# decisiongraph/duckdb-annsearch

Hardware: AMD Instinct MI355X
Metric: queries/sec @ recall@10>=0.95, 10Mx768 fp32, batch=1024 (higher is better)
Workload: dtype f32 results (fp16-image certified filter + exact fp32 rerank); 1 GPU; FAISS IVFFlat nlist=1024 nprobe=32, 10000000x768 fp32 (low-rank gaussian, intrinsic dim 16, noise 0.02), batch=1024, k=10; global_batch=1024, n=10000000, d=768, k=10, parallelism=shard1

## Files before the change

### duckdb-annsearch_amd/csrc/ivf.cpp

```cpp
#include "../../include/hip_ann.h"
#include "ivf.hpp"

#include <algorithm>
#include <chrono>
#include <cstdio>
#include <cstdlib>
#include <cstring>
#include <exception>
#include <numeric>

using namespace hipann;

namespace {

void set_err(char *buf, int len, const char *msg) {
    if (!buf || len <= 0) return;
    std::strncpy(buf, msg, (size_t)len - 1);
    buf[len - 1] = '\0';
}

template <typename F>
int guard_int(char *eb, int el, F &&f) {
    try {
        return f();
// ... 471 lines not shown
    int *cand_i = nullptr;
    const float *qn = nullptr;
    if (form != kFormDirect && metric == kL2) {
        const FlatShard &qs = *sh.quant->shards[0];
        if (probes_in && img) {
            qn = qsh0.qn.get<float>();
        } else if (!probes_in && qs.qn_of == xq && qs.qn_nq == nq) {
            qn = qs.qn.get<float>();
        } else {
            sh.qn.ensure(sizeof(float) * (size_t)nq, sh.device);
            launch_row_norms(xq, nq, d, sh.qn.get<float>(), st);
            qn = sh.qn.get<float>();
        }
    }
    if (tiled && !img) ensure_tiled_codes(sh, d, nlist, st);
    if (img) {
    } else if (ivf_form_split(form)) {
        sh.qsplit.ensure((size_t)ivf_mfma_bf_qsplit_bytes(nq, d, ivf_form_terms(form)), sh.device);
    }
    {
        RoctxRange rr("hipann.ivf.scan");
        ScopedTiming t(ix.timer_main, st);
        if (img) {
            auto scan_h = [&](int phase, const int *slots, int64_t items, float *pd, int *pi, int subl) {
                launch_ivf_scan_mfma_h(nq, i8 ? sh.qi8.p : sh.hsplit.p, i8 ? sh.qs8.get<float>() : sh.hits.get<float>(),
                                       i8 ? sh.qres8.get<float>() : sh.hres.get<float>(), cert8 ? sh.qhn2.get<float>() : qn, d,
                                       metric, i8 ? sh.codes_i8.p : sh.codes_h.p, sh.tpass_off.get<int64_t>(), sh.xnorm.get<float>(),
                                       sh.list_off.get<int64_t>(), sh.list_len.get<int>(), sh.cnt.get<int>(), sh.bucket_off.get<int>(),
                                       sh.item_off.get<int>(), sh.bucket.get<int>(), slots, nlist, np, k,
                                       items, qbound, pd, pi, st, subl,
                                       i8 ? 1 : 0, i8 ? sh.xs8.get<float>() : nullptr,
                                       cert8 ? sh.xr8.get<float>() : nullptr, cert8 ? sh.qhn.get<float>() : nullptr, phase,
                                       sh.goff.get<int>());
            };
            if (seeded) {
                HIPANN_REQUIRE((int64_t)np * nq * sh.max_nch + nq < (int64_t)0x7fffffff, "too many candidate slots");
                sh.cslot.ensure(sizeof(int) * (size_t)nq * np, sh.device);
                sh.bcnt.ensure(sizeof(int) * (size_t)nq, sh.device);
                cand_d = sh.part_d.get<float>() + (size_t)np * nq * kslot;
                cand_i = sh.part_i.get<int>() + (size_t)np * nq * kslot;
                scan_h(1, nullptr, ivf_max_items(nq, np, nlist, 1, 0, group), sh.part_d.get<float>(), sh.part_i.get<int>(), 1);
                launch_ivf_seed_bound(sh.part_d.get<float>(), sh.part_i.get<int>(), sh.slot_off.get<int>(), np, nq, kslot,
                                      sh.n, qbound, cand_d, cand_i, sh.cslot.get<int>(), sh.bcnt.get<int>(), st);
                scan_h(2, sh.cslot.get<int>(), ivf_max_items(nq, np, nlist, sh.max_nch - 1, sh.n, group), cand_d, cand_i, 1);
            } else {
                scan_h(0, sh.slot_off.get<int>(), max_items, sh.part_d.get<float>(), sh.part_i.get<int>(), sub ? 1 : 0);
            }
        }
        else if (bigk)
            launch_ivf_scan_bigk(xq, d, metric, sh.codes, sh.list_off.get<int64_t>(), sh.list_len.get<int>(),
                                 sh.coarse_i.get<int64_t>(),
                                 nq * np, np, sh.slot_off.get<int>(), nq * np * std::max(sh.max_nch, 1), k,
                                 sh.part_d.get<float>(), sh.part_i.get<int>(), st);
        else if (ivf_form_split(form))
            launch_ivf_scan_mfma_bf(ivf_form_terms(form), xq, nq, sh.qsplit.p, qn, d, metric, sh.codes_t.get<float>(),
                                    sh.tpass_off.get<int64_t>(), sh.xnorm.get<float>(), sh.list_off.get<int64_t>(),
                                    sh.list_len.get<int>(), sh.cnt.get<int>(), sh.bucket_off.get<int>(), sh.item_off.get<int>(),
                                    sh.bucket.get<int>(), sh.slot_off.get<int>(), nlist, np, k, max_items, qbound,
                                    sh.part_d.get<float>(), sh.part_i.get<int>(), st, sub ? 1 : 0);
        else if (form == kFormDecomposed)
            launch_ivf_scan_mfma(xq, qn, d, metric, sh.codes_t.get<float>(), sh.tpass_off.get<int64_t>(),
                                 sh.xnorm.get<float>(), sh.list_off.get<int64_t>(), sh.list_len.get<int>(),
                                 sh.cnt.get<int>(),
                                 sh.bucket_off.get<int>(), sh.item_off.get<int>(), sh.bucket.get<int>(),
                                 sh.slot_off.get<int>(), nlist, np, k, max_items, qbound, sh.part_d.get<float>(),
                                 sh.part_i.get<int>(), st);
        else
// ... 20 lines not shown
        fb_maxch = sh.max_nch;
        const size_t per_f = (size_t)np * fb_maxch * kout * (sizeof(float) + sizeof(long long));
        fb_cap = (int)std::min<int64_t>({nq, 64, std::max<int64_t>(1, (int64_t)(((size_t)64 << 20) / per_f))});
        sh.fbc_d.ensure(sizeof(float) * (size_t)fb_cap * np * fb_maxch * kout, sh.device);
        sh.fbc_i.ensure(sizeof(long long) * (size_t)fb_cap * np * fb_maxch * kout, sh.device);
        if (sh.fbc_cap < fb_cap || !sh.fbc_done.p) {
            sh.fbc_done.ensure(sizeof(unsigned) * (size_t)std::max(fb_cap, 64), sh.device);
            HIPANN_CHECK(hipMemsetAsync(sh.fbc_done.p, 0, sh.fbc_done.bytes, st));
            sh.fbc_cap = (int)(sh.fbc_done.bytes / sizeof(unsigned));
        }
    }
    {
        RoctxRange rr("hipann.ivf.rerank");
        ScopedTiming t(ix.timer_merge, st);
        launch_ivf_rerank(seeded ? cand_d : sh.part_d.get<float>(), seeded ? cand_i : sh.part_i.get<int>(),
                          sh.slot_off.get<int>(), np, nq, kfilt, kout,
                          metric, xq, sh.codes, d, sh.ids, sh.n, 0, xmax2, D, I, sh.nflag.get<int>(),
                          sh.flagged.get<int>(), st, kSplit2Eps, i8 ? rxmax8 : half ? sh.half_rxmax : -1.f,
                          i8 ? sh.qres8.get<float>() : half ? sh.hres.get<float>() : nullptr, sh.coarse_i.get<int64_t>(),
                          sh.list_off.get<int64_t>(), nlist, qbound, img && metric == kL2 ? qn : nullptr, kslot,
                          sub ? 1 : 0, inline_fb ? sh.list_len.get<int>() : nullptr,
                          inline_fb ? sh.fpd.get<float>() : nullptr, inline_fb ? sh.fpi.get<long long>() : nullptr,
                          inline_fb ? sh.fb_total.get<unsigned long long>() : nullptr, fb_cap, cert8 ? 1 : 0,
                          seeded ? sh.bcnt.get<int>() : nullptr);
        if (fb_cap > 0)
            launch_ivf_fallback_chunks(sh.nflag.get<int>(), sh.flagged.get<int>(), fb_cap, np, fb_maxch, ivf_chunk_rows(),
                                       kout, metric, xq, sh.codes, d, sh.ids, 0, sh.coarse_i.get<int64_t>(),
                                       sh.list_off.get<int64_t>(), sh.list_len.get<int>(), nlist, sh.fbc_d.get<float>(),
                                       sh.fbc_i.get<long long>(), sh.fbc_done.get<unsigned>(), D, I,
                                       sh.fb_total.get<unsigned long long>(), st,
                                       as_half && !probation ? auto8_host_word(sh) : nullptr, (unsigned)++sh.fb_seq);
    }
    if (sh.count_only) return;
    if (probation) auto8_probation(ix, sh, nq, xq, k_user, kout, st, probes_in);
    if (inline_fb) return;
    int nf = 0;
    HIPANN_CHECK(hipMemcpyAsync(&nf, sh.nflag.p, sizeof(int), hipMemcpyDeviceToHost, st));
    HIPANN_CHECK(hipStreamSynchronize(st));
    if (nf <= 0) return;
    ix.rerank_fallbacks += nf;
    const size_t pbytes = sizeof(int64_t) * (size_t)nq * np;
    sh.coarse_save.ensure(pbytes, sh.device);
    HIPANN_CHECK(hipMemcpyAsync(sh.coarse_save.p, sh.coarse_i.p, pbytes, hipMemcpyDeviceToDevice, st));
    sh.fq.ensure(sizeof(float) * (size_t)nf * d, sh.device);
    sh.fD.ensure(sizeof(float) * (size_t)nf * kout, sh.device);
    sh.fI.ensure(sizeof(int64_t) * (size_t)nf * kout, sh.device);
    launch_ivf_gather_queries(xq, sh.flagged.get<int>(), nf, d, sh.fq.get<float>(), st);
// ... 834 lines not shown
```

### duckdb-annsearch_amd/csrc/ivf_kernels.hip

```cpp
#include "common.hpp"
#include "wave_topk.hpp"

#include <algorithm>
#include <cstdlib>
#include <utility>

namespace hipann {

constexpr int IVF_WAVES = 8;
constexpr int IVF_THREADS = 64 * IVF_WAVES;
constexpr int IVF_G = 32;
constexpr int IVF_QW = IVF_G / IVF_WAVES;
constexpr int IVF_TR = 256;
constexpr int IVF_BK = 24;
constexpr int IVF_LD = IVF_BK + 4;
#ifndef HIPANN_IVF_CH
#define HIPANN_IVF_CH 2048
#endif
constexpr int IVF_CH = HIPANN_IVF_CH;

__device__ __forceinline__ int ivf_nch(int len) { return (len + IVF_CH - 1) / IVF_CH; }

__global__ void ivf_count(const int64_t *__restrict__ probes, int64_t npairs, const int *__restrict__ list_len,
                          int nlist, int *__restrict__ cnt) {
// ... 1775 lines not shown
#endif
template <bool IP, int WV>
__global__ void __launch_bounds__(WV == 1 ? 256 : 64 * WV, WV == 4 ? HIPANN_RR_MINB : 1)
ivf_rerank_topk(const float *__restrict__ pd, const int *__restrict__ pi, const int *__restrict__ slot_off,
                int nprobe, int64_t nq, int k, int kout, const float *__restrict__ Q,
                const float *__restrict__ codes, int d, const int64_t *__restrict__ ids, int64_t nrows,
                int64_t label_offset, float xmax2, float *__restrict__ D, int64_t *__restrict__ I,
                int *__restrict__ nflag, int *__restrict__ flagged, float eps, float rxmax,
                const float *__restrict__ qres, const int64_t *__restrict__ probes,
                const int64_t *__restrict__ list_off, int nlist, const unsigned *__restrict__ qbound,
                const float *__restrict__ qnorm, int kslot, int sub, const int *__restrict__ list_len,
                float *__restrict__ fpd, long long *__restrict__ fpi, unsigned long long *__restrict__ fb_total,
                int fb_cap, int i8_l2, const int *__restrict__ seed_cnt) {
    const int64_t q = WV == 1 ? (int64_t)blockIdx.x * 4 + (threadIdx.x >> 6) : (int64_t)blockIdx.x;
    if (q >= nq) return;
    const int lane = threadIdx.x & 63;
    const int wv = WV == 1 ? 0 : (int)(threadIdx.x >> 6);
    RR_STAMP(0);
    long long rr_t = HIPANN_RR_PROF ? clock64() : 0;
    WaveList<1, int> L;
    L.init();
    const int64_t s0 = slot_off ? slot_off[q * nprobe] : q * nprobe;
    const int64_t s1 = slot_off ? slot_off[(q + 1) * nprobe] : (q + 1) * nprobe;
    const int64_t total = seed_cnt ? kSeedK + (int64_t)seed_cnt[q] * kslot : (s1 - s0) * kslot;
    const int64_t first = seed_cnt ? (ivf_seed_run_slot((int)s0, q) + 1) * kslot - kSeedK : s0 * kslot;
    if constexpr (HIPANN_RR_STAMP != 0) { if (total >= 0) RR_STAMP(1); }
    pd += first;
    pi += first;
    float tsub = __builtin_inff();
    if (sub && qbound) {
        const unsigned b = qbound[q];
        const float t = __uint_as_float((b & 0x80000000u) ? (b & 0x7fffffffu) : ~b);
        tsub = t == t ? t : __builtin_inff();
    }
    constexpr int RS_J = 16;
    const bool bsel = WV > 1 && total <= (int64_t)64 * WV * RS_J && !rerank_lists();
    if (WV > 1 && !bsel) RR_COUNT(9);
    constexpr int MU = 4;
    for (int64_t cb = (int64_t)wv * 64; !bsel && cb < total; cb += 64 * WV * MU) {
        float vv[MU];
        int rr[MU];
#pragma unroll
        for (int u = 0; u < MU; ++u) {
            const int64_t c = cb + (int64_t)u * 64 * WV + lane;
            vv[u] = c < total ? pd[c] : __builtin_inff();
            rr[u] = c < total ? pi[c] : -1;
        }
// ... 349 lines not shown

__global__ void __launch_bounds__(256) ivf_gather_queries(const float *__restrict__ Q, const int *__restrict__ idx, int nf,
                                                          int d, float *__restrict__ out) {
    const int64_t t = (int64_t)blockIdx.x * 256 + threadIdx.x;
    if (t >= (int64_t)nf * d) return;
    const int j = (int)(t / d), e = (int)(t - (int64_t)j * d);
    out[t] = Q[(int64_t)idx[j] * d + e];
}

__global__ void __launch_bounds__(256) ivf_scatter_results(const float *__restrict__ Df, const int64_t *__restrict__ If,
                                                           const int *__restrict__ idx, int nf, int kout,
                                                           float *__restrict__ D, int64_t *__restrict__ I) {
    const int64_t t = (int64_t)blockIdx.x * 256 + threadIdx.x;
    if (t >= (int64_t)nf * kout) return;
    const int j = (int)(t / kout), e = (int)(t - (int64_t)j * kout);
    D[(int64_t)idx[j] * kout + e] = Df[t];
    I[(int64_t)idx[j] * kout + e] = If[t];
}

constexpr int kSeedWaves = 4, kSeedJ = 16;
__global__ void __launch_bounds__(64 * kSeedWaves)
ivf_seed_bound(const float *__restrict__ pa_d, const int *__restrict__ pa_i, const int *__restrict__ slot_off, int nprobe,
               int64_t nq, int kslot, int64_t nrows, unsigned *__restrict__ qbound, float *__restrict__ cd,
               int *__restrict__ ci, int *__restrict__ cslot, int *__restrict__ bcnt) {
    const int64_t q = blockIdx.x;
    if (q >= nq) return;
    const int lane = threadIdx.x & 63, wv = threadIdx.x >> 6;
    const int64_t p0 = q * nprobe;
    const int64_t s0 = ivf_seed_run_slot(slot_off[p0], q);
    if (wv == 0) {
        int carry = 0;
        for (int pb = 0; pb < nprobe; pb += 64) {
            const int p = pb + lane;
            const int nch = p < nprobe ? slot_off[p0 + p + 1] - slot_off[p0 + p] : 0;
            const int nb = ivf_seed_pair_slots(nch);
            int x = nb;
#pragma unroll
            for (int o = 1; o < 64; o <<= 1) {
                const int t = __shfl_up(x, o);
                if (lane >= o) x += t;
            }
            if (p < nprobe) cslot[p0 + p] = (int)(s0 + 1 + carry + x - nb);
            carry += __shfl(x, 63);
        }
        if (lane == 0) bcnt[q] = carry;
    }
    const unsigned b = qbound[q];
    const float t = __uint_as_float((b & 0x80000000u) ? (b & 0x7fffffffu) : ~b);
    const float bound = t == t ? t : __builtin_inff();
    __shared__ float wk[kSeedWaves * 64 * kSeedJ], sk[kSeedWaves * 64], ntk[kSeedWaves * 64];
    __shared__ int wp[kSeedWaves * 64 * kSeedJ], sp[kSeedWaves * 64], ntp[kSeedWaves * 64];
    __shared__ int scnt[kSeedWaves];
    WaveList<1, int> L;
    L.init();
    bool bad = false;
    long long rr_t = 0;
    rerank_wave_select<kSeedWaves, kSeedJ>(pa_d + p0 * kslot, pa_i + p0 * kslot, (int64_t)nprobe * kslot, kSeedK, nrows,
                                           bound, wk, wp, sk, sp, scnt, L, bad, rr_t, q, ntk, ntp, slot_off + p0, kslot);
    if (wv != 0) return;
    const bool real = L.id[0] != IdTraits<int>::pad();
    cd[(s0 + 1) * kslot - kSeedK + lane] = real ? L.d[0] : __builtin_inff();
    ci[(s0 + 1) * kslot - kSeedK + lane] = L.id[0];
    if (lane == kSeedK - 1 && real) {
        const unsigned u = __float_as_uint(L.d[0]);
        atomicMin(qbound + q, (u & 0x80000000u) ? ~u : (u | 0x80000000u));
    }
}

extern "C" int hipann_debug_ivf_seed_items(const int *list_len, const int *cnt, int nlist, int group, int *item_off,
// ... 18 lines not shown
            out[3 * item] = l;
            out[3 * item + 1] = chunk;
            out[3 * item + 2] = grp;
        }
    }
    return 0;
}
extern "C" void hipann_debug_ivf_seed_slots(const int *slot_off, int nprobe, int64_t nq, int64_t *cslot, int *bcnt) {
    for (int64_t q = 0; q < nq; ++q) {
        int64_t s = ivf_seed_run_slot(slot_off[q * nprobe], q) + 1;
        for (int p = 0; p < nprobe; ++p) {
            cslot[q * nprobe + p] = s;
            s += ivf_seed_pair_slots(slot_off[q * nprobe + p + 1] - slot_off[q * nprobe + p]);
        }
        bcnt[q] = (int)(s - ivf_seed_run_slot(slot_off[q * nprobe], q) - 1);
    }
}

bool ivf_seed_supported(int nprobe, int kslot) {
    return nprobe >= 1 && kslot >= kSeedK && (int64_t)nprobe * kslot <= (int64_t)64 * kSeedWaves * kSeedJ;
}

void launch_ivf_seed_bound(const float *pa_d, const int *pa_i, const int *slot_off, int nprobe, int64_t nq, int kslot,
                           int64_t nrows, unsigned *qbound, float *cd, int *ci, int *cslot, int *bcnt, hipStream_t st) {
    if (nq <= 0) return;
    HIPANN_REQUIRE(ivf_seed_supported(nprobe, kslot) && nq < (int64_t)0x7fffffff, "ivf seed bound: too many chunk-0 entries");
    static_assert(kSeedK == 64, "the seed list is one wave wide");
    hipLaunchKernelGGL(ivf_seed_bound, dim3((unsigned)nq), dim3(64 * kSeedWaves), 0, st, pa_d, pa_i, slot_off, nprobe, nq,
                       kslot, nrows, qbound, cd, ci, cslot, bcnt);
    HIPANN_CHECK(hipGetLastError());
}

#ifndef HIPANN_RR_WIDE
#define HIPANN_RR_WIDE (1 << 30)
#endif

void launch_ivf_rerank(const float *pd, const int *pi, const int *slot_off, int nprobe, int64_t nq, int k, int kout,
                       int metric, const float *Q, const float *codes, int d, const int64_t *ids, int64_t nrows,
                       int64_t label_offset, float xmax2, float *D, int64_t *I, int *nflag, int *flagged,
                       hipStream_t st, float eps, float rxmax, const float *qres, const int64_t *probes,
                       const int64_t *list_off, int nlist, const unsigned *qbound, const float *qnorm, int kslot,
                       int sub, const int *list_len, float *fpd, long long *fpi, unsigned long long *fb_total,
                       int fb_cap, int i8_l2, const int *seed_cnt) {
    if (nq <= 0) return;
    if (kslot <= 0) kslot = k;
    HIPANN_REQUIRE(!seed_cnt || (slot_off && sub && qbound), "ivf rerank: candidate runs need the slot table and the bound");
    HIPANN_REQUIRE(!i8_l2 || (metric == kL2 && qres && qnorm), "ivf rerank: the int8 L2 certificate needs ‖q − q̂‖ and ‖q‖²");
    HIPANN_REQUIRE(k >= kRerankK && k <= 64 && kout >= 1 && kout <= k && kslot >= 1 && (!sub || qbound),
                   "ivf rerank: k / kout out of range");
    HIPANN_REQUIRE(!fpd || (fpi && list_len && probes && list_off && fb_total), "ivf rerank: inline re-run buffers");
    const bool wide = nq < HIPANN_RR_WIDE;
    dim3 grid((unsigned)(wide ? nq : ceil_div(nq, 4))), block(256);
// ... 63 lines not shown
```

### duckdb-annsearch_amd/csrc/ivf_mfma.hip

```cpp
#include "common.hpp"
#include "wave_topk.hpp"

#include <algorithm>
#include <cstdio>
#include <cstdlib>
#include <cstring>

namespace hipann {

typedef float mf_f32x4 __attribute__((ext_vector_type(4)));

#ifndef HIPANN_MF_EXPERIMENT
#define HIPANN_MF_EXPERIMENT 0
#endif

#ifndef HIPANN_MF_WAVES
#define HIPANN_MF_WAVES 8
#endif
#ifndef HIPANN_MF_P
#define HIPANN_MF_P 6
#endif
#ifndef HIPANN_MF_QPF
#define HIPANN_MF_QPF 0
#endif
// ... 92 lines not shown
#pragma unroll
    for (int r = 0; r < 4; ++r) {
        rl[r] = (unsigned)__builtin_amdgcn_readlane((int)lo, 16 * r + kth);
        rh[r] = (unsigned)__builtin_amdgcn_readlane((int)hi, 16 * r + kth);
    }
    const unsigned sl = g == 0 ? rl[0] : g == 1 ? rl[1] : g == 2 ? rl[2] : rl[3];
    const unsigned sh = g == 0 ? rh[0] : g == 1 ? rh[1] : g == 2 ? rh[2] : rh[3];
    return ((uint64_t)sh << 32) | sl;
}

__device__ __forceinline__ unsigned row_kth_key(uint64_t l, int kth, int g) {
    const unsigned hi = (unsigned)(l >> 32);
    unsigned rh[4];
#pragma unroll
    for (int r = 0; r < 4; ++r) rh[r] = (unsigned)__builtin_amdgcn_readlane((int)hi, 16 * r + kth);
    return g == 0 ? rh[0] : g == 1 ? rh[1] : g == 2 ? rh[2] : rh[3];
}

template <int QT>
__device__ __forceinline__ void mf_finish_item(uint64_t (&lst)[QT][4], float *smem, int nqi,
                                               const int *__restrict__ bucket, int boff, int nprobe,
                                               const int *__restrict__ slot_off, int chunk, int k, int sub,
                                               unsigned *__restrict__ qbound, float *__restrict__ part_d,
                                               int *__restrict__ part_i) {
    const int lane = threadIdx.x & 63;
    const int wave = __builtin_amdgcn_readfirstlane(threadIdx.x >> 6);
    const int m = lane & 15, g = lane >> 4;
    if (!sub) {
        uint64_t *scratch = reinterpret_cast<uint64_t *>(smem);
#pragma unroll 1
        for (int half = MF_WAVES / 2; half > 0; half >>= 1) {
            __syncthreads();
            if (wave >= half && wave < 2 * half) {
                uint64_t *dst = scratch + (size_t)(wave - half) * QT * 4 * 64;
#pragma unroll
                for (int qt = 0; qt < QT; ++qt)
#pragma unroll
                    for (int v = 0; v < 4; ++v) dst[(qt * 4 + v) * 64 + lane] = lst[qt][v];
            }
            __syncthreads();
            if (wave < half) {
                const uint64_t *src = scratch + (size_t)wave * QT * 4 * 64;
#pragma unroll
                for (int qt = 0; qt < QT; ++qt)
#pragma unroll
                    for (int v = 0; v < 4; ++v) row_merge16(lst[qt][v], src[(qt * 4 + v) * 64 + lane], m);
            }
        }
    }
    if ((sub || wave == 0) && m < k) {
// ... 1033 lines not shown
        out[((q * 2 + 1) * nsup + S) * 4 + gg] = make_uint4(lw[0], lw[1], lw[2], lw[3]);
    }
#pragma unroll
    for (int o = 32; o > 0; o >>= 1) {
        r2 += __shfl_xor(r2, o);
        r1 += __shfl_xor(r1, o);
    }
    if (lane == 0) {
        its[q] = ldexpf(1.f, ok ? eits : 0);
        qres[q] = ok ? sqrtf(r2) * 1.0001f : __builtin_inff();
        qres[nq + q] = ok ? sqrtf(r1) * 1.0001f : __builtin_inff();
    }
}

template <int QT, bool IP, bool I8>
__device__ __forceinline__ void mh_item(int d, const uint4 *__restrict__ codes_h, int64_t tp0,
                                        const float *__restrict__ xn, int64_t r0, int64_t r1, int nqi,
                                        const unsigned *__restrict__ qs, int stride, const unsigned (&qb)[QT][4],
                                        const float *__restrict__ qpar,
                                        const int *__restrict__ bucket, int boff, int nprobe,
                                        const int *__restrict__ slot_off, int chunk, int k, int sub, float *smem,
                                        unsigned *__restrict__ qbound, float *__restrict__ part_d,
                                        int *__restrict__ part_i, const float *__restrict__ xs8,
                                        const float *__restrict__ xr8, int stat_part) {
    const int lane = threadIdx.x & 63;
    const int wave = __builtin_amdgcn_readfirstlane(threadIdx.x >> 6);
    const int m = lane & 15, g = lane >> 4;
    const int nsup = I8 ? mi_nsup(d) : mh_nsup(d);
    const int npass_all = (int)ceil_div(r1 - r0, MF_PASS);
    const int npass = npass_all > wave ? (npass_all - wave + MF_WAVES - 1) / MF_WAVES : 0;

    uint64_t lst[QT][4];
    unsigned thr[QT][4];
#pragma unroll
    for (int qt = 0; qt < QT; ++qt)
#pragma unroll
        for (int v = 0; v < 4; ++v) {
            const uint64_t b = ((uint64_t)qb[qt][v] << 32) | MF_PAD_ID;
            lst[qt][v] = m < k ? b : MF_EMPTY;
            thr[qt][v] = qb[qt][v];
        }

    auto row_of = [&](int i, int r) -> int64_t {
        const int64_t row = r0 + (int64_t)(wave + MF_WAVES * i) * MF_PASS + 16 * r + m;
        return row < r1 ? row : r1 - 1;
    };
    const int ilast = npass > 0 ? npass - 1 : 0;
// ... 149 lines not shown
                        thr[qt][v] = row_kth_key(lst[qt][v], k - 1, g);
                    }
                }
        }
#pragma unroll
        for (int r = 0; r < MF_RT; ++r) {
            xnr[r] = xnr_next[r];
            xsr[r] = xsr_next[r];
            xrr[r] = xrr_next[r];
        }
    }

    if (HIPANN_MF_EXPERIMENT == 1 && sink == 1) part_d[0] = 0.f;
#if HIPANN_MH_STATS
    if (lane == 0) {
        unsigned long long *st = mh_stats_dev[I8][stat_part];
        atomicAdd(st + 0, (unsigned long long)npass);
        atomicAdd(st + 1, (unsigned long long)st_step);
        atomicAdd(st + 2, (unsigned long long)st_hit);
        atomicAdd(st + 3, (unsigned long long)st_rows);
        atomicAdd(st + 4, (unsigned long long)st_ins);
    }
#endif
    mf_finish_item<QT>(lst, smem, nqi, bucket, boff, nprobe, slot_off, chunk, k, sub, qbound, part_d, part_i);
}

template <int TS>
__device__ __forceinline__ void mh_fill(unsigned *qs, const uint4 *__restrict__ qsplit, int nsup, int stride, int nqi,
                                        const int *__restrict__ bucket, int boff, int nprobe) {
    const int per_q = nsup * 4;
    for (int t = threadIdx.x; t < nqi * per_q; t += MF_THREADS) {
        const int q = t / per_q, r2 = t - q * per_q;
        const int gq = bucket[boff + q] / nprobe;
        *reinterpret_cast<uint4 *>(qs + q * stride + r2 * 4) = qsplit[(int64_t)gq * TS * nsup * 4 + r2];
    }
}

template <bool IP, bool I8>
__global__ void __launch_bounds__(MF_THREADS, MF_WAVES / 4)
ivf_scan_mfma_h(const uint4 *__restrict__ qsplit, const float *__restrict__ qnorm, const float *__restrict__ its, int d,
                const uint4 *__restrict__ codes_h, const int64_t *__restrict__ tpass_off, const float *__restrict__ xn,
                const int64_t *__restrict__ list_off, const int *__restrict__ list_len, const int *__restrict__ cnt, const int *__restrict__ bucket_off,
                const int *__restrict__ item_off, const int *__restrict__ bucket, const int *__restrict__ slot_off,
                int nlist, int nprobe, int group, int k, int sub, unsigned *__restrict__ qbound, float *__restrict__ part_d,
                int *__restrict__ part_i, float *__restrict__ qres, int nq, int remap, const float *__restrict__ xs8,
                const float *__restrict__ xr8, const float *__restrict__ qhn, int phase, const int *__restrict__ goff) {
    extern __shared__ __attribute__((aligned(16))) float smem[];
    const int total = ivf_phase_first(phase, item_off[nlist], phase ? goff[nlist] : 0);
    if ((int)blockIdx.x >= total) return;
    const int item = remap ? xcd_remap((int)blockIdx.x, total) : (int)blockIdx.x;
    const int l = ivf_phase_list(phase, item_off, goff, nlist, item);
    const int64_t lr0 = list_off[l], lr1 = lr0 + list_len[l];
    const int c = cnt[l];
    const int ng = ivf_ngroups(c, group);
    int chunk, grp;
    ivf_phase_decode(phase, item - ivf_phase_first(phase, item_off[l], phase ? goff[l] : 0), ng, chunk, grp);
    const int slot_chunk = phase == 2 ? chunk - 1 : chunk;
    const int q_begin = (int)((int64_t)grp * c / ng), q_end = (int)((int64_t)(grp + 1) * c / ng);
    const int nqi = q_end - q_begin;
    const int64_t r0 = lr0 + (int64_t)chunk * MF_CH;
    const int64_t r1 = r0 + MF_CH < lr1 ? r0 + MF_CH : lr1;
    const int boff = bucket_off[l] + q_begin;
    const int nqt = (nqi + 15) >> 4;

    const int64_t tp0 = tpass_off[l] + (int64_t)chunk * (MF_CH / MF_PASS);
    unsigned *qs = reinterpret_cast<unsigned *>(smem);
    const int nsup = I8 ? mi_nsup(d) : mh_nsup(d);
    const int stride = I8 ? mi_nsup(d) * 16 + 8 : mh_stride(d);
    float *qpar = reinterpret_cast<float *>(qs + nqi * stride);
    mh_fill<I8 ? 1 : 2>(qs, qsplit, nsup, stride, nqi, bucket, boff, nprobe);
    for (int t = threadIdx.x; t < nqi; t += MF_THREADS) {
        const int qi = bucket[boff + t] / nprobe;
        if constexpr (I8)
            reinterpret_cast<float4 *>(qpar)[t] =
                make_float4(IP ? 0.f : qnorm[qi], its[qi], IP ? 0.f : 2.f * qhn[qi], 0.f);
        else reinterpret_cast<float2 *>(qpar)[t] = make_float2(IP ? 0.f : qnorm[qi], its[qi]);
        if (!I8) qres[qi] = qres[nq + qi];
    }

    const int lane = threadIdx.x & 63, g = lane >> 4;
    const int stat_part = phase ? 1 + phase : (int64_t)blockIdx.x * 5 < (int64_t)total ? 0 : 1;
#define MH_CASE(QTV)                                                                                        \
    {                                                                                                       \
        unsigned qb[QTV][4];                                                                                \
        _Pragma("unroll") for (int qt = 0; qt < QTV; ++qt) _Pragma("unroll") for (int v = 0; v < 4; ++v) {  \
            const int q = qt * 16 + 4 * g + v;                                                              \
            const int qi = q < nqi ? bucket[boff + q] / nprobe : 0;                                         \
            qb[qt][v] = q < nqi ? __atomic_load_n(qbound + qi, __ATOMIC_RELAXED) : 0xffffffffu;             \
        }                                                                                                   \
        mh_item<QTV, IP, I8>(d, codes_h, tp0, xn, r0, r1, nqi, qs, stride, qb, qpar, bucket, boff, nprobe, slot_off, \
                             slot_chunk, k, sub, smem, qbound, part_d, part_i, xs8, xr8, stat_part);        \
    }
    switch (nqt) {
    case 0: case 1: MH_CASE(1) break;
    case 2: MH_CASE(2) break;
    case 3: MH_CASE(3) break;
    case 4: MH_CASE(4) break;
    case 5: MH_CASE(5) break;
    default: MH_CASE(6) break;
    }
#undef MH_CASE
}

void ivf_mh_stats_report() {
#if HIPANN_MH_STATS
    unsigned long long h[2][4][5];
    static const char *const names[4] = {"first_fifth", "rest", "seeded_chunk0", "seeded_rest"};
    if (hipMemcpyFromSymbol(h, HIP_SYMBOL(mh_stats_dev), sizeof(h)) != hipSuccess) return;
    for (int i8 = 0; i8 < 2; ++i8)
        for (int part = 0; part < 4; ++part)
            std::fprintf(stderr, "HIPANN_MH_STATS image=%s blocks=%s passes=%llu steps=%llu hit_steps=%llu admitted_rows=%llu "
                                 "insert_steps=%llu\n", i8 ? "int8" : "fp16", names[part], h[i8][part][0],
                         h[i8][part][1], h[i8][part][2], h[i8][part][3], h[i8][part][4]);
    std::memset(h, 0, sizeof(h));
// ... 68 lines not shown
    int64_t blocks = std::max(ceil_div(n, (int64_t)4), ceil_div((int64_t)nlist, (int64_t)256));
    if (!dst) blocks = std::min<int64_t>(blocks, 64);
    HIPANN_REQUIRE(blocks < (int64_t)0x7fffffff, "append block too large");
    if (stat) HIPANN_CHECK(hipMemsetAsync(stat, 0, sizeof(unsigned) * 4, st));
    hipLaunchKernelGGL(ivf_append_rows, dim3((unsigned)blocks), dim3(256), 0, st, rows, norms, dst, ids_in, n, d, codes,
                       ids, xnorm, newlen, list_len, nlist, hscale, stat);
    HIPANN_CHECK(hipGetLastError());
}

void launch_ivf_split_queries_h(const float *Q, int64_t nq, int d, int es, void *qsplit, float *its, float *qres,
                                float *qn, hipStream_t st) {
    if (nq <= 0) return;
    const int vec4 = (d % 4 == 0) && ((uintptr_t)Q % 16 == 0);
    hipLaunchKernelGGL(ivf_split_queries_h, dim3((unsigned)ceil_div(nq, 4)), dim3(256), 0, st, Q, nq, d, mh_nsup(d), es,
                       static_cast<uint4 *>(qsplit), its, qres, qn, vec4);
    HIPANN_CHECK(hipGetLastError());
}

void launch_ivf_scan_mfma_h(int64_t nq, const void *qsplit, const float *its, float *qres, const float *qn, int d,
                            int metric, const void *codes_h, const int64_t *tpass_off, const float *xn,
                            const int64_t *list_off, const int *list_len, const int *cnt, const int *bucket_off,
                            const int *item_off, const int *bucket, const int *slot_off, int nlist, int nprobe, int k,
                            int64_t max_items, unsigned *qbound, float *pd, int *pi, hipStream_t st, int sub, int i8mode,
                            const float *xs8, const float *xr8, const float *qhn, int phase, const int *goff) {
    if (max_items <= 0 || nq <= 0) return;
    HIPANN_REQUIRE(phase == 0 ? slot_off != nullptr : goff && (phase == 1) == (slot_off == nullptr),
                   "fp16 / int8 IVF scan: phase 1 writes pair slots, phase 2 needs the pairs' chunk-1 slots");
    HIPANN_REQUIRE(max_items < (int64_t)0x7fffffff, "too many IVF work items");
    HIPANN_REQUIRE(qsplit && its && qres && codes_h, "fp16 IVF scan: missing buffers");
    HIPANN_REQUIRE(i8mode ? ivf_mfma_i8_supported(d, k) && xs8 : ivf_mfma_h_supported(d, k),
                   "fp16 / int8 IVF scan needs k <= 16 (int8: scales and prepared queries)");
    HIPANN_REQUIRE(metric == kIP || (qn && xn), "decomposed L2 scan needs query and row norms");
    HIPANN_REQUIRE(!i8mode || metric == kIP || (xr8 && qhn), "int8 L2 scan needs the rows' residuals and the queries' norms");
    const uint4 *qs = static_cast<const uint4 *>(qsplit);
    const int group = i8mode ? ivf_mfma_i8_group(d) : mh_group_packed(d);
    const size_t merge = (size_t)(MF_WAVES / 2) * MH_QTW * 4 * 64 * sizeof(float2);
    const size_t per_q = i8mode ? (size_t)(mi_nsup(d) * 16 + 8) * 4 + 16 : (size_t)mh_stride(d) * 4 + 8;
    const size_t smem = std::max((size_t)ivf_group_wide(group) * per_q, merge);
    HIPANN_REQUIRE(smem <= MF_LDS_MAX, "fp16 IVF scan: LDS image too large");
    HIPANN_REQUIRE(nq < (int64_t)0x7fffffff, "fp16 IVF scan: batch too large");
    dim3 grid((unsigned)max_items), block(MF_THREADS);
    const uint4 *ch = static_cast<const uint4 *>(codes_h);
    static const int remap = [] { const char *e = std::getenv("HIPANN_IVF_REMAP"); return !e || std::atoi(e) ? 1 : 0; }();
#define MH_LAUNCH_ARGS qs, qn, its, d, ch, tpass_off, xn, list_off, list_len, cnt, bucket_off, item_off, bucket, slot_off, nlist, nprobe, \
                       group, k, sub, qbound, pd, pi, qres, (int)nq, remap, xs8, xr8, qhn, phase, goff
    if (i8mode) {
        if (metric == kIP) hipLaunchKernelGGL((ivf_scan_mfma_h<true, true>), grid, block, smem, st, MH_LAUNCH_ARGS);
        else hipLaunchKernelGGL((ivf_scan_mfma_h<false, true>), grid, block, smem, st, MH_LAUNCH_ARGS);
    } else {
        if (metric == kIP) hipLaunchKernelGGL((ivf_scan_mfma_h<true, false>), grid, block, smem, st, MH_LAUNCH_ARGS);
        else hipLaunchKernelGGL((ivf_scan_mfma_h<false, false>), grid, block, smem, st, MH_LAUNCH_ARGS);
    }
#undef MH_LAUNCH_ARGS
    HIPANN_CHECK(hipGetLastError());
}

}
```

### duckdb-annsearch_amd/csrc/runtime.hpp

```cpp
#pragma once
#include "common.hpp"
#include <cstdlib>
#include <ctime>
#include <memory>
#include <mutex>
#include <vector>

namespace hipann {

struct DeviceGuard {
    int prev = 0;
    explicit DeviceGuard(int dev) {
        HIPANN_CHECK(hipGetDevice(&prev));
        if (prev != dev) HIPANN_CHECK(hipSetDevice(dev));
    }
    ~DeviceGuard() { (void)hipSetDevice(prev); }
};

struct DevBuf {
    void *p = nullptr;
    size_t bytes = 0;
    int device = 0;
    DevBuf() = default;
    DevBuf(const DevBuf &) = delete;
// ... 282 lines not shown
        int64_t b = 0;
        for (auto &s : shards)
            b += s->n * (int64_t)d * 4 + (metric == kL2 ? s->n * 4 : 0) + (int64_t)s->xb16.bytes +
                 (int64_t)s->xi8.bytes + (int64_t)s->xscale.bytes;
        return b;
    }
};

struct IvfShard {
    int device = 0;
    int64_t n = 0;
    int64_t live = 0;
    const float *centroids = nullptr;
    const float *codes = nullptr;
    const int64_t *ids = nullptr;
    DevBuf centroids_buf, codes_buf, ids_buf;
    DevBuf list_off;
    DevBuf list_len;
    DevBuf xnorm;
    std::unique_ptr<FlatIndex> quant;
    hipStream_t stream = nullptr;
    DevBuf q, qn, coarse_d, coarse_i, cnt, bucket_off, item_off, cursor, bucket, slot_off, part_d, part_i, out_d, out_i;
    DevBuf qbound;
    DevBuf goff, cslot, bcnt;
    DevBuf qsplit;
    float xmax2 = -1.f;
    DevBuf nflag, flagged, fq, fD, fI, coarse_save, tmpnorm;
    DevBuf ccnt, qtot;
    DevBuf cursor2;
    uint64_t plan_batch = 0;
    int plan_nlist = 0;
    DevBuf fpd, fpi;
    DevBuf fb_total;
    DevBuf fbc_d, fbc_i, fbc_done;
    int fbc_cap = 0;
    std::vector<int64_t> h_off;
    std::vector<int64_t> h_len;
    bool owns_codes = false;
    DevBuf codes_t, tpass_off;
    int half_state = 0, half_es = 0;
    float half_rxmax = 0.f;
    DevBuf codes_h, hsplit, hits, hres;
    int i8_state = 0;
    float i8_rxmax = -1.f;
    int64_t i8_tiled = 0;
    DevBuf codes_i8, xs8, xr8, qi8, qs8, qres8, qhn2, qhn;
    int auto8 = 0, auto8_over = 0;
// ... 101 lines not shown
                                int kout, int metric, const float *Q, const float *codes, int d, const int64_t *ids,
                                int64_t label_offset, const int64_t *probes, const int64_t *list_off,
                                const int *list_len, int nlist, float *cpd, long long *cpi, unsigned *done, float *D,
                                int64_t *I, unsigned long long *total, hipStream_t st,
                                unsigned long long *host_word = nullptr, unsigned host_seq = 0);
int ivf_mfma_h_group(int d);
void ivf_mh_stats_report();
int ivf_scan_sublists();
int64_t ivf_half_pass_bytes(int d);
int64_t ivf_half_qsplit_bytes(int64_t nq, int d);
bool ivf_mfma_h_supported(int d, int k);
void launch_ivf_max_abs(const float *x, int64_t cnt, unsigned *out, hipStream_t st);
void launch_ivf_tile_half(const float *codes, const int64_t *list_off, const int *list_len, const int64_t *tpass_off,
                          int nlist, int64_t total_pass, int d, float scale, void *dst, hipStream_t st,
                          const int64_t *pass_ids = nullptr);
void launch_ivf_half_residual(const float *codes, int64_t n, int d, float scale, unsigned *out, hipStream_t st);
void launch_ivf_scan_mfma_h(int64_t nq, const void *qsplit, const float *its, float *qres, const float *qn, int d,
                            int metric, const void *codes_h, const int64_t *tpass_off, const float *xn,
                            const int64_t *list_off, const int *list_len, const int *cnt, const int *bucket_off,
                            const int *item_off, const int *bucket, const int *slot_off, int nlist, int nprobe, int k,
                            int64_t max_items, unsigned *qbound, float *pd, int *pi, hipStream_t st, int sub = 0,
                            int i8mode = 0, const float *xs8 = nullptr, const float *xr8 = nullptr,
                            const float *qhn = nullptr,
                            int phase = 0, const int *goff = nullptr);
bool ivf_seed_supported(int nprobe, int kslot);
void launch_ivf_seed_bound(const float *pa_d, const int *pa_i, const int *slot_off, int nprobe, int64_t nq, int kslot,
                           int64_t nrows, unsigned *qbound, float *cd, int *ci, int *cslot, int *bcnt, hipStream_t st);
int ivf_mfma_i8_group(int d);
int64_t ivf_i8_pass_bytes(int d);
int64_t ivf_i8_qimg_bytes(int64_t nq, int d);
bool ivf_mfma_i8_supported(int d, int k);
void launch_ivf_tile_i8(const float *codes, const int64_t *list_off, const int *list_len, const int64_t *tpass_off,
                        int nlist, int64_t total_pass, int d, void *dst, float *xs8, float *xr8, unsigned *nonfin,
                        hipStream_t st, const int64_t *pass_ids = nullptr);
void launch_ivf_split_queries_i8(const float *Q, int64_t nq, int d, void *qi8, float *qs8, float *qres8,
                                 float *qhn2, float *qhn, hipStream_t st);
void launch_ivf_split_queries_h(const float *Q, int64_t nq, int d, int es, void *qsplit, float *its, float *qres,
                                float *qn, hipStream_t st);
int flat_bf16_waves(int64_t nq);
int flat_bf16_tile_rows();
int flat_bf16_topk_kmax(int64_t nq);
int flat_gemm_topk_bf_kmax(int np);
size_t flat_bf16_img_bytes(int64_t n, int d, int R);
void launch_b16_tile_rows(const float *X, int64_t n, int d, int R, void *out, hipStream_t st);
void launch_b16_row_residual2(const float *X, int64_t n, int d, float *out, hipStream_t st);
void launch_flat_bf16_topk(const float *Q, const float *qn, int64_t nq, void *qimg, const void *ximg, const float *xn,
                           int64_t N, int d, int metric, int k, int nsplit, int64_t tiles_per_split, float *pd, int *pi,
                           const float *seed, bool image_ready, hipStream_t st);
bool flat_bf16_resumable(int64_t nq, int d, int k);
void launch_flat_bf16_k64(const void *qimg, const float *qn, int64_t nq, const void *ximg, const float *xn, int64_t N,
// ... 84 lines not shown
```

Before: 568,200 queries/s.

## Append phase-2 int8 scan candidates through per-query atomic cursors

Phase 2 of the seeded int8 IVF scan no longer writes a fixed k-slot block per (query, chunk) pair. Each wave now uses an atomicAdd on a per-query cursor to compact only its real surviving candidates into one contiguous run per query. The seed-bound kernel drops its prefix-sum over pair slots and just resets the cursor, and rerank reads the compacted count instead of count times kslot. This cuts rerank input size and the pad/empty entries it must skip, at the cost of atomic contention, a nondeterministic candidate order, and an opt-in debug stats path that syncs to the host.

```diff
diff --git a/duckdb-annsearch_amd/csrc/ivf.cpp b/duckdb-annsearch_amd/csrc/ivf.cpp
--- a/duckdb-annsearch_amd/csrc/ivf.cpp
+++ b/duckdb-annsearch_amd/csrc/ivf.cpp
@@ -517,7 +517,8 @@
         RoctxRange rr("hipann.ivf.scan");
         ScopedTiming t(ix.timer_main, st);
         if (img) {
-            auto scan_h = [&](int phase, const int *slots, int64_t items, float *pd, int *pi, int subl) {
+            auto scan_h = [&](int phase, const int *slots, int64_t items, float *pd, int *pi, int subl,
+                              int *run_cnt = nullptr) {
                 launch_ivf_scan_mfma_h(nq, i8 ? sh.qi8.p : sh.hsplit.p, i8 ? sh.qs8.get<float>() : sh.hits.get<float>(),
                                        i8 ? sh.qres8.get<float>() : sh.hres.get<float>(), cert8 ? sh.qhn2.get<float>() : qn, d,
                                        metric, i8 ? sh.codes_i8.p : sh.codes_h.p, sh.tpass_off.get<int64_t>(), sh.xnorm.get<float>(),
@@ -526,18 +527,30 @@
                                        items, qbound, pd, pi, st, subl,
                                        i8 ? 1 : 0, i8 ? sh.xs8.get<float>() : nullptr,
                                        cert8 ? sh.xr8.get<float>() : nullptr, cert8 ? sh.qhn.get<float>() : nullptr, phase,
-                                       sh.goff.get<int>());
+                                       sh.goff.get<int>(), run_cnt);
             };
             if (seeded) {
                 HIPANN_REQUIRE((int64_t)np * nq * sh.max_nch + nq < (int64_t)0x7fffffff, "too many candidate slots");
-                sh.cslot.ensure(sizeof(int) * (size_t)nq * np, sh.device);
-                sh.bcnt.ensure(sizeof(int) * (size_t)nq, sh.device);
+                HIPANN_REQUIRE((int64_t)np * sh.max_nch * kslot < (int64_t)0x7fffffff, "candidate run too long");
+                sh.run_cnt.ensure(sizeof(int) * (size_t)nq, sh.device);
                 cand_d = sh.part_d.get<float>() + (size_t)np * nq * kslot;
                 cand_i = sh.part_i.get<int>() + (size_t)np * nq * kslot;
                 scan_h(1, nullptr, ivf_max_items(nq, np, nlist, 1, 0, group), sh.part_d.get<float>(), sh.part_i.get<int>(), 1);
                 launch_ivf_seed_bound(sh.part_d.get<float>(), sh.part_i.get<int>(), sh.slot_off.get<int>(), np, nq, kslot,
-                                      sh.n, qbound, cand_d, cand_i, sh.cslot.get<int>(), sh.bcnt.get<int>(), st);
-                scan_h(2, sh.cslot.get<int>(), ivf_max_items(nq, np, nlist, sh.max_nch - 1, sh.n, group), cand_d, cand_i, 1);
+                                      sh.n, qbound, cand_d, cand_i, sh.run_cnt.get<int>(), st);
+                scan_h(2, sh.slot_off.get<int>(), ivf_max_items(nq, np, nlist, sh.max_nch - 1, sh.n, group), cand_d, cand_i, 1,
+                       sh.run_cnt.get<int>());
+                static const bool run_stats = [] { const char *e = std::getenv("HIPANN_IVF_RUN_STATS"); return e && std::atoi(e) != 0; }();
+                if (run_stats) {
+                    std::vector<int> h((size_t)nq);
+                    HIPANN_CHECK(hipMemcpyAsync(h.data(), sh.run_cnt.p, sizeof(int) * (size_t)nq, hipMemcpyDeviceToHost, st));
+                    HIPANN_CHECK(hipStreamSynchronize(st));
+                    int64_t sum = 0, over = 0;
+                    int mx = 0;
+                    for (int c : h) { sum += c; mx = std::max(mx, c); over += kSeedK + c > 4096; }
+                    std::fprintf(stderr, "HIPANN_IVF_RUN_STATS nq=%lld appended_total=%lld mean=%.1f max=%d runs_over_4096=%lld\n",
+                                 (long long)nq, (long long)sum, (double)sum / (double)nq, mx, (long long)over);
+                }
             } else {
                 scan_h(0, sh.slot_off.get<int>(), max_items, sh.part_d.get<float>(), sh.part_i.get<int>(), sub ? 1 : 0);
             }
@@ -604,7 +617,7 @@
                           sub ? 1 : 0, inline_fb ? sh.list_len.get<int>() : nullptr,
                           inline_fb ? sh.fpd.get<float>() : nullptr, inline_fb ? sh.fpi.get<long long>() : nullptr,
                           inline_fb ? sh.fb_total.get<unsigned long long>() : nullptr, fb_cap, cert8 ? 1 : 0,
-                          seeded ? sh.bcnt.get<int>() : nullptr);
+                          seeded ? sh.run_cnt.get<int>() : nullptr);
         if (fb_cap > 0)
             launch_ivf_fallback_chunks(sh.nflag.get<int>(), sh.flagged.get<int>(), fb_cap, np, fb_maxch, ivf_chunk_rows(),
                                        kout, metric, xq, sh.codes, d, sh.ids, 0, sh.coarse_i.get<int64_t>(),
diff --git a/duckdb-annsearch_amd/csrc/ivf_kernels.hip b/duckdb-annsearch_amd/csrc/ivf_kernels.hip
--- a/duckdb-annsearch_amd/csrc/ivf_kernels.hip
+++ b/duckdb-annsearch_amd/csrc/ivf_kernels.hip
@@ -1821,7 +1821,7 @@
     L.init();
     const int64_t s0 = slot_off ? slot_off[q * nprobe] : q * nprobe;
     const int64_t s1 = slot_off ? slot_off[(q + 1) * nprobe] : (q + 1) * nprobe;
-    const int64_t total = seed_cnt ? kSeedK + (int64_t)seed_cnt[q] * kslot : (s1 - s0) * kslot;
+    const int64_t total = seed_cnt ? kSeedK + (int64_t)seed_cnt[q] : (s1 - s0) * kslot;
     const int64_t first = seed_cnt ? (ivf_seed_run_slot((int)s0, q) + 1) * kslot - kSeedK : s0 * kslot;
     if constexpr (HIPANN_RR_STAMP != 0) { if (total >= 0) RR_STAMP(1); }
     pd += first;
@@ -2217,29 +2217,13 @@
 __global__ void __launch_bounds__(64 * kSeedWaves)
 ivf_seed_bound(const float *__restrict__ pa_d, const int *__restrict__ pa_i, const int *__restrict__ slot_off, int nprobe,
                int64_t nq, int kslot, int64_t nrows, unsigned *__restrict__ qbound, float *__restrict__ cd,
-               int *__restrict__ ci, int *__restrict__ cslot, int *__restrict__ bcnt) {
+               int *__restrict__ ci, int *__restrict__ cursor) {
     const int64_t q = blockIdx.x;
     if (q >= nq) return;
     const int lane = threadIdx.x & 63, wv = threadIdx.x >> 6;
     const int64_t p0 = q * nprobe;
     const int64_t s0 = ivf_seed_run_slot(slot_off[p0], q);
-    if (wv == 0) {
-        int carry = 0;
-        for (int pb = 0; pb < nprobe; pb += 64) {
-            const int p = pb + lane;
-            const int nch = p < nprobe ? slot_off[p0 + p + 1] - slot_off[p0 + p] : 0;
-            const int nb = ivf_seed_pair_slots(nch);
-            int x = nb;
-#pragma unroll
-            for (int o = 1; o < 64; o <<= 1) {
-                const int t = __shfl_up(x, o);
-                if (lane >= o) x += t;
-            }
-            if (p < nprobe) cslot[p0 + p] = (int)(s0 + 1 + carry + x - nb);
-            carry += __shfl(x, 63);
-        }
-        if (lane == 0) bcnt[q] = carry;
-    }
+    if (threadIdx.x == 0) cursor[q] = 0;
     const unsigned b = qbound[q];
     const float t = __uint_as_float((b & 0x80000000u) ? (b & 0x7fffffffu) : ~b);
     const float bound = t == t ? t : __builtin_inff();
@@ -2304,12 +2288,12 @@
 }
 
 void launch_ivf_seed_bound(const float *pa_d, const int *pa_i, const int *slot_off, int nprobe, int64_t nq, int kslot,
-                           int64_t nrows, unsigned *qbound, float *cd, int *ci, int *cslot, int *bcnt, hipStream_t st) {
+                           int64_t nrows, unsigned *qbound, float *cd, int *ci, int *cursor, hipStream_t st) {
     if (nq <= 0) return;
     HIPANN_REQUIRE(ivf_seed_supported(nprobe, kslot) && nq < (int64_t)0x7fffffff, "ivf seed bound: too many chunk-0 entries");
     static_assert(kSeedK == 64, "the seed list is one wave wide");
     hipLaunchKernelGGL(ivf_seed_bound, dim3((unsigned)nq), dim3(64 * kSeedWaves), 0, st, pa_d, pa_i, slot_off, nprobe, nq,
-                       kslot, nrows, qbound, cd, ci, cslot, bcnt);
+                       kslot, nrows, qbound, cd, ci, cursor);
     HIPANN_CHECK(hipGetLastError());
 }
 
diff --git a/duckdb-annsearch_amd/csrc/ivf_mfma.hip b/duckdb-annsearch_amd/csrc/ivf_mfma.hip
--- a/duckdb-annsearch_amd/csrc/ivf_mfma.hip
+++ b/duckdb-annsearch_amd/csrc/ivf_mfma.hip
@@ -138,10 +138,37 @@
                                                const int *__restrict__ bucket, int boff, int nprobe,
                                                const int *__restrict__ slot_off, int chunk, int k, int sub,
                                                unsigned *__restrict__ qbound, float *__restrict__ part_d,
-                                               int *__restrict__ part_i) {
+                                               int *__restrict__ part_i, int *__restrict__ cursor = nullptr) {
     const int lane = threadIdx.x & 63;
     const int wave = __builtin_amdgcn_readfirstlane(threadIdx.x >> 6);
     const int m = lane & 15, g = lane >> 4;
+    if (cursor) {
+#pragma unroll
+        for (int qt = 0; qt < QT; ++qt)
+#pragma unroll
+            for (int v = 0; v < 4; ++v) {
+                const int q = qt * 16 + 4 * g + v;
+                const uint64_t e = lst[qt][v];
+                const unsigned id = (unsigned)e;
+                const bool real = q < nqi && m < k && e != MF_EMPTY && id != MF_PAD_ID;
+                const uint64_t rm = __ballot(real);
+                if (rm) {
+                    const int n = __popc((unsigned)(rm >> (16 * g)) & 0xffffu);
+                    const int qi = n ? bucket[boff + q] / nprobe : 0;
+                    int base = 0;
+                    if (m == 0 && n) base = atomicAdd(cursor + qi, n);
+                    base = __shfl(base, lane & 48);
+                    if (m < n) {
+                        const int64_t off =
+                            (ivf_seed_run_slot(slot_off[(int64_t)qi * nprobe], qi) + 1) * (MF_WAVES * k) + base + m;
+                        part_d[off] = mf_unsortable((unsigned)(e >> 32));
+                        part_i[off] = (int)id;
+                        if (m == k - 1) atomicMin(qbound + qi, (unsigned)(e >> 32));
+                    }
+                }
+            }
+        return;
+    }
     if (!sub) {
         uint64_t *scratch = reinterpret_cast<uint64_t *>(smem);
 #pragma unroll 1
@@ -1221,7 +1248,7 @@
                                         const int *__restrict__ slot_off, int chunk, int k, int sub, float *smem,
                                         unsigned *__restrict__ qbound, float *__restrict__ part_d,
                                         int *__restrict__ part_i, const float *__restrict__ xs8,
-                                        const float *__restrict__ xr8, int stat_part) {
+                                        const float *__restrict__ xr8, int stat_part, int *__restrict__ cursor) {
     const int lane = threadIdx.x & 63;
     const int wave = __builtin_amdgcn_readfirstlane(threadIdx.x >> 6);
     const int m = lane & 15, g = lane >> 4;
@@ -1417,7 +1444,7 @@
         atomicAdd(st + 4, (unsigned long long)st_ins);
     }
 #endif
-    mf_finish_item<QT>(lst, smem, nqi, bucket, boff, nprobe, slot_off, chunk, k, sub, qbound, part_d, part_i);
+    mf_finish_item<QT>(lst, smem, nqi, bucket, boff, nprobe, slot_off, chunk, k, sub, qbound, part_d, part_i, cursor);
 }
 
 template <int TS>
@@ -1439,7 +1466,8 @@
                 const int *__restrict__ item_off, const int *__restrict__ bucket, const int *__restrict__ slot_off,
                 int nlist, int nprobe, int group, int k, int sub, unsigned *__restrict__ qbound, float *__restrict__ part_d,
                 int *__restrict__ part_i, float *__restrict__ qres, int nq, int remap, const float *__restrict__ xs8,
-                const float *__restrict__ xr8, const float *__restrict__ qhn, int phase, const int *__restrict__ goff) {
+                const float *__restrict__ xr8, const float *__restrict__ qhn, int phase, const int *__restrict__ goff,
+                int *__restrict__ cursor) {
     extern __shared__ __attribute__((aligned(16))) float smem[];
     const int total = ivf_phase_first(phase, item_off[nlist], phase ? goff[nlist] : 0);
     if ((int)blockIdx.x >= total) return;
@@ -1450,7 +1478,6 @@
     const int ng = ivf_ngroups(c, group);
     int chunk, grp;
     ivf_phase_decode(phase, item - ivf_phase_first(phase, item_off[l], phase ? goff[l] : 0), ng, chunk, grp);
-    const int slot_chunk = phase == 2 ? chunk - 1 : chunk;
     const int q_begin = (int)((int64_t)grp * c / ng), q_end = (int)((int64_t)(grp + 1) * c / ng);
     const int nqi = q_end - q_begin;
     const int64_t r0 = lr0 + (int64_t)chunk * MF_CH;
@@ -1484,7 +1511,8 @@
             qb[qt][v] = q < nqi ? __atomic_load_n(qbound + qi, __ATOMIC_RELAXED) : 0xffffffffu;             \
         }                                                                                                   \
         mh_item<QTV, IP, I8>(d, codes_h, tp0, xn, r0, r1, nqi, qs, stride, qb, qpar, bucket, boff, nprobe, slot_off, \
-                             slot_chunk, k, sub, smem, qbound, part_d, part_i, xs8, xr8, stat_part);        \
+                             chunk, k, sub, smem, qbound, part_d, part_i, xs8, xr8, stat_part,         \
+                             I8 && !IP ? cursor : nullptr);                                                 \
     }
     switch (nqt) {
     case 0: case 1: MH_CASE(1) break;
@@ -1599,10 +1627,13 @@
                             const int64_t *list_off, const int *list_len, const int *cnt, const int *bucket_off,
                             const int *item_off, const int *bucket, const int *slot_off, int nlist, int nprobe, int k,
                             int64_t max_items, unsigned *qbound, float *pd, int *pi, hipStream_t st, int sub, int i8mode,
-                            const float *xs8, const float *xr8, const float *qhn, int phase, const int *goff) {
+                            const float *xs8, const float *xr8, const float *qhn, int phase, const int *goff,
+                            int *cursor) {
     if (max_items <= 0 || nq <= 0) return;
     HIPANN_REQUIRE(phase == 0 ? slot_off != nullptr : goff && (phase == 1) == (slot_off == nullptr),
-                   "fp16 / int8 IVF scan: phase 1 writes pair slots, phase 2 needs the pairs' chunk-1 slots");
+                   "fp16 / int8 IVF scan: phase 1 writes pair slots, phase 2 needs the plan's slot prefixes");
+    HIPANN_REQUIRE((phase == 2) == (cursor != nullptr) && (!cursor || (i8mode && metric == kL2 && sub)),
+                   "int8 IVF scan: phase 2 (int8 image, L2, sub-lists) appends through the queries' cursors");
     HIPANN_REQUIRE(max_items < (int64_t)0x7fffffff, "too many IVF work items");
     HIPANN_REQUIRE(qsplit && its && qres && codes_h, "fp16 IVF scan: missing buffers");
     HIPANN_REQUIRE(i8mode ? ivf_mfma_i8_supported(d, k) && xs8 : ivf_mfma_h_supported(d, k),
@@ -1620,7 +1651,7 @@
     const uint4 *ch = static_cast<const uint4 *>(codes_h);
     static const int remap = [] { const char *e = std::getenv("HIPANN_IVF_REMAP"); return !e || std::atoi(e) ? 1 : 0; }();
 #define MH_LAUNCH_ARGS qs, qn, its, d, ch, tpass_off, xn, list_off, list_len, cnt, bucket_off, item_off, bucket, slot_off, nlist, nprobe, \
-                       group, k, sub, qbound, pd, pi, qres, (int)nq, remap, xs8, xr8, qhn, phase, goff
+                       group, k, sub, qbound, pd, pi, qres, (int)nq, remap, xs8, xr8, qhn, phase, goff, cursor
     if (i8mode) {
         if (metric == kIP) hipLaunchKernelGGL((ivf_scan_mfma_h<true, true>), grid, block, smem, st, MH_LAUNCH_ARGS);
         else hipLaunchKernelGGL((ivf_scan_mfma_h<false, true>), grid, block, smem, st, MH_LAUNCH_ARGS);
diff --git a/duckdb-annsearch_amd/csrc/runtime.hpp b/duckdb-annsearch_amd/csrc/runtime.hpp
--- a/duckdb-annsearch_amd/csrc/runtime.hpp
+++ b/duckdb-annsearch_amd/csrc/runtime.hpp
@@ -328,7 +328,7 @@
     hipStream_t stream = nullptr;
     DevBuf q, qn, coarse_d, coarse_i, cnt, bucket_off, item_off, cursor, bucket, slot_off, part_d, part_i, out_d, out_i;
     DevBuf qbound;
-    DevBuf goff, cslot, bcnt;
+    DevBuf goff, run_cnt;
     DevBuf qsplit;
     float xmax2 = -1.f;
     DevBuf nflag, flagged, fq, fD, fI, coarse_save, tmpnorm;
@@ -476,10 +476,10 @@
                             int64_t max_items, unsigned *qbound, float *pd, int *pi, hipStream_t st, int sub = 0,
                             int i8mode = 0, const float *xs8 = nullptr, const float *xr8 = nullptr,
                             const float *qhn = nullptr,
-                            int phase = 0, const int *goff = nullptr);
+                            int phase = 0, const int *goff = nullptr, int *cursor = nullptr);
 bool ivf_seed_supported(int nprobe, int kslot);
 void launch_ivf_seed_bound(const float *pa_d, const int *pa_i, const int *slot_off, int nprobe, int64_t nq, int kslot,
-                           int64_t nrows, unsigned *qbound, float *cd, int *ci, int *cslot, int *bcnt, hipStream_t st);
+                           int64_t nrows, unsigned *qbound, float *cd, int *ci, int *cursor, hipStream_t st);
 int ivf_mfma_i8_group(int d);
 int64_t ivf_i8_pass_bytes(int d);
 int64_t ivf_i8_qimg_bytes(int64_t nq, int d);
```

Result: faster. 612,900 queries/s (median of 6 runs) (+7.9%).
